# TheShinning/gps-sdr-sim

Hardware: AMD Instinct MI355X
Metric: IQ MSamples/s (and × real-time) at 2.6 MS/s, 12 sats, -b 16; 1/2/4/8 GPU (higher is better)
Workload: dtype int64 phases + f16 x f16 -> f32 MFMA accumulate (exact integer sums)

## Files before the change

### gps-sdr-sim_amd/csrc/hip/gss_synth.hip

```cpp
#include <hip/hip_runtime.h>
#include <stdint.h>
#include <stdlib.h>
#include <string.h>
#include "gpssim_amd.h"
#include "../common/gss_phase.h"
#include "../common/gss_lin.h"

#define SYNTH_THREADS  256
#define SYNTH_WAVES    (SYNTH_THREADS / 64)
#define ANCHOR_THREADS 64
#define CHUNK_BYTES    128
#define CHUNK_PIECES   (CHUNK_BYTES / 16)
#define LUT_N          1024

struct lut_arg { int16_t sin512[512]; int16_t cos512[512]; };

__global__ __launch_bounds__(ANCHOR_THREADS) void gss_anchor_kernel(
    const gss_chan_blk_t *__restrict__ blk, const int32_t *__restrict__ nch,
    const double *__restrict__ carr_ck, int nblk, int nchp, int n_per_blk, int nseg, int nsegp,
    int seg_r, double *__restrict__ seg_carr, double *__restrict__ seg_code,
    uint32_t *__restrict__ seg_cnt, double *__restrict__ carr_end,
    const int32_t *__restrict__ blist)
{
    const int nsub = carr_ck ? GSS_NCK : 1;
// ... 322 lines not shown
            } else {
                bits = (bits << 2) | ((uint32_t)(i16 > 0) << 1) | (uint32_t)(q16 > 0);
                if ((sidx & 15) == 15) {
                    int nb = nsamp - (sidx & ~15);
                    uint32_t w32 = nb >= 16 ? bits : nb > 0 ? (bits >> 2 * (16 - nb)) << 2 * (16 - nb) : 0u;
                    mine[sidx >> 4] = __builtin_bswap32(w32);
                    bits = 0;
                }
            }
        }
        if (last_seg && full && (ch + 1) * SPC == len) {
#pragma unroll
            for (int k = 0; k < NCH; k++) {
                const uint32_t c = s_st[k][tid];
                bad |= (C[k] >= GSS_CA_SEQ_LEN_D && c == (19u | (29u << 5) | (59u << 10))) ? 1 : 0;
            }
        }
        const bool any_full = __any(full);
        if (any_full) {
            wave_sync_lds();
            for (int i = 0; i < CHUNK_PIECES; i++) {
                int src = (64 / CHUNK_PIECES) * i + lane / CHUNK_PIECES, piece = lane % CHUNK_PIECES;
                int src_full = __shfl(full ? 1 : 0, src);
                if (src_full) {
                    uint8_t *sdst = dst + (ptrdiff_t)(src - lane) * ((ptrdiff_t)seg_r * BPS4 / 4) +
                                    (size_t)ch * CHUNK_BYTES + piece * 16;
                    const uint32_t *sp = stg + src * (CHUNK_BYTES / 4) + piece * 4;
                    store16(sdst, make_uint4(sp[0], sp[1], sp[2], sp[3]));
                }
            }
            wave_sync_lds();
        }
        if (!full && nsamp > 0) {
            int nbytes = nsamp * BPS4 / 4;
            uint8_t *bp = dst + (size_t)ch * CHUNK_BYTES;
            const uint8_t *sp = (const uint8_t *)mine;
            for (int i = 0; i < nbytes; i++)
                bp[i] = sp[i];
        }
    }
    if (bad && status)
        atomicOr(status, bad);
}

#define LIN_THREADS 256
#define LIN_WAVES   (LIN_THREADS / 64)
#define LIN_STEPS   (GSS_LIN_SEG / 64)
#define LIN_CH      GSS_LIN_CH
#define CBW_PRE     2
#define CBW_CHIPS   3072
#define CAB_W       ((CBW_CHIPS + 96) / 32)
static_assert(LIN_STEPS % LIN_CH == 0 && (LIN_CH & (LIN_CH - 1)) == 0, "whole chunks");
#define LIN_SW_SGPRS 68
typedef _Float16 lin_half4 __attribute__((ext_vector_type(4)));
typedef _Float16 lin_half8 __attribute__((ext_vector_type(8)));
typedef float lin_f4 __attribute__((ext_vector_type(4)));
#define LIN_GS    2
#define LIN_MAGF  (12582912.0f + 64.0f * LIN_GS)
#define LIN_MAGB  0x4B400000u

struct alignas(16) lin_ct {
    uint64_t B;
    uint64_t D;
    int32_t g;
    int32_t gd;
    int32_t pos1;
    uint32_t flags;
    uint32_t q0, dq, tab;
    uint32_t wa;
    uint32_t na, nb;
    uint32_t wn;
    uint32_t g2;
    uint32_t A[5][2];
};
static_assert(offsetof(lin_ct, A) % 8 == 0, "lin_ct.A: 8-byte reads");

typedef gss_lin_row lin_seg;
typedef gss_lin_chan lin_chan;
static_assert(sizeof(lin_seg) == 32 && sizeof(lin_chan) == 32, "two 16-byte LDS reads each");

__global__ void gss_cab_kernel(const uint32_t *__restrict__ ca_bits, int n_ca,
                               uint32_t *__restrict__ cab)
{
    const int i = blockIdx.x * blockDim.x + threadIdx.x;
    if (i >= n_ca * CAB_W)
        return;
    const int row = i / CAB_W, j0 = (i - row * CAB_W) * 32 - 32;
    const uint32_t *cb = ca_bits + (size_t)row * GSS_CA_WORDS;
    uint32_t w = 0;
    for (int q = 0; q < 32; q++) {
        const int e = j0 + q, chip = ((e % GSS_CA_LEN) + GSS_CA_LEN) % GSS_CA_LEN;
        w |= (((cb[chip >> 5] >> (chip & 31)) & 1u) ^ 1u) << q;
    }
    cab[i] = w;
}

__global__ void gss_tw16_kernel(const uint32_t *__restrict__ cab, int n_ca, uint32_t w,
                                uint32_t *__restrict__ tw)
{
    const int i = blockIdx.x * blockDim.x + threadIdx.x;
    if (i >= n_ca * GSS_LIN_TWE * LIN_CH)
        return;
    const int row = i / (GSS_LIN_TWE * LIN_CH), r = i - row * (GSS_LIN_TWE * LIN_CH);
    const int E = r / LIN_CH, st = r % LIN_CH;
    const uint32_t j = min((uint32_t)(E + (int)(((uint32_t)st * w) >> 4) - GSS_LIN_CBW_PRE + 32),
                           (uint32_t)(32 * CAB_W - 64));
    const uint32_t *c = cab + (size_t)row * CAB_W;
    const uint32_t lin = __builtin_amdgcn_alignbit(c[(j >> 5) + 1], c[j >> 5], j & 31);
    tw[i] = __builtin_amdgcn_alignbit(lin, lin, (32u - j) & 31u);
}

struct lin_wsrc {
    const uint32_t *W;
};

__device__ __forceinline__ void lin_wissue(const lin_wsrc &w, uint32_t (&ws)[LIN_CH])
{
#pragma unroll
    for (int s = 0; s < LIN_CH; s++)
        ws[s] = w.W[s];
}

__device__ __forceinline__ void lin_wfence(const uint32_t (&ws)[LIN_CH])
{
    static_assert(LIN_CH == 16, "the fence below names 16 windows");
// ... 135 lines not shown
{
    const lin_ct &ta = T[k0], &tb = T[k0 + 1];
    uint64_t Pa = s_lane[k0 * 64 + lane] + ta.B, Pb = s_lane[(k0 + 1) * 64 + lane] + tb.B;
    const uint64_t Da = ta.D, Db = tb.D;
    const uint2 ga = *(const uint2 *)ta.A[cls], gb = *(const uint2 *)tb.A[cls];
    const lin_half8 A = __builtin_bit_cast(lin_half8, make_uint4(ga.x, ga.y, gb.x, gb.y));
    uint32_t na = ta.na, nb = ta.nb;
    asm volatile("" : "+v"(na), "+v"(nb));
    uint32_t wsa[LIN_CH], wsb[LIN_CH];
    lin_sw_take_a(wsa);
    lin_sw_take(wsb);
    if (k0 + 2 < nc || more)
        lin_sw_load2(tw, na, nb);
    uint32_t ea0 = 0, eb0 = 0;
#pragma unroll
    for (int s = 0; s < LIN_CH; s++) {
        uint32_t ta_, tb_;
        asm("v_lshrrev_b32_sdwa %0, %1, %2 dst_sel:DWORD dst_unused:UNUSED_PAD src0_sel:BYTE_3 "
            "src1_sel:DWORD" : "=v"(ta_) : "v"((uint32_t)Pa), "s"(wsa[s]));
        asm("v_lshrrev_b32_sdwa %0, %1, %2 dst_sel:DWORD dst_unused:UNUSED_PAD src0_sel:BYTE_3 "
            "src1_sel:DWORD" : "=v"(tb_) : "v"((uint32_t)Pb), "s"(wsb[s]));
        const uint32_t aa = __builtin_amdgcn_alignbit(ta_, (uint32_t)(Pa >> 32), 21) & M;
        const uint32_t ab = __builtin_amdgcn_alignbit(tb_, (uint32_t)(Pb >> 32), 21) & M;
        const uint32_t ea = *(const uint32_t *)((const char *)s_lut + aa);
        const uint32_t eb = *(const uint32_t *)((const char *)s_lut + ab);
        if (s & 1) {
            const uint4 bb = make_uint4(ea0, ea, eb0, eb);
            cq[s / 2] = __builtin_amdgcn_mfma_f32_16x16x32_f16(A, __builtin_bit_cast(lin_half8, bb),
                                                              FIRST ? c0 : cq[s / 2], 0, 0, 0);
        } else {
            ea0 = ea;
            eb0 = eb;
        }
        Pa += Da;
        Pb += Db;
    }
}

__device__ __forceinline__ lin_half4 lin_gain_operand(uint32_t gh, int lane)
{
    const uint32_t x = gh << ((lane & 1) * 16);
    const uint2 v = (lane & 2) ? make_uint2(0u, x) : make_uint2(x, 0u);
    return __builtin_bit_cast(lin_half4, v);
}

__host__ __device__ __forceinline__ uint32_t lin_f16_bits(int g)
{
    return (uint32_t)__builtin_bit_cast(uint16_t, (_Float16)(float)g);
}

__device__ __forceinline__ void lin_put(uint32_t *p, uint32_t v)
{
    __builtin_nontemporal_store(v, p);
}

extern "C" __device__ int gss_writelane(int, int, int) __asm("llvm.amdgcn.writelane.i32");

__device__ __forceinline__ uint32_t lin_ib(const lin_f4 (&cq)[LIN_CH / 2], int s)
{
    return __float_as_uint(cq[s / 2][2 * (s & 1)]);
}
__device__ __forceinline__ uint32_t lin_qb(const lin_f4 (&cq)[LIN_CH / 2], int s)
{
    return __float_as_uint(cq[s / 2][2 * (s & 1) + 1]);
}
__device__ __forceinline__ uint32_t lin_w16(const lin_f4 (&cq)[LIN_CH / 2], int s)
{
    const uint32_t pq = __builtin_amdgcn_perm(lin_qb(cq, s), lin_ib(cq, s), 0x06050201u);
    uint32_t r;
    asm("v_pk_add_u16 %0, %1, %2" : "=v"(r) : "v"(pq), "s"(0xC000C000u));
    return r;
}
__device__ __forceinline__ uint32_t lin_w8(const lin_f4 (&cq)[LIN_CH / 2], int s)
{
    constexpr uint32_t sh = 12u;
    uint32_t d = lin_ib(cq, s) >> sh;
    asm("v_lshrrev_b32_sdwa %0, %1, %2 dst_sel:BYTE_1 dst_unused:UNUSED_PRESERVE src0_sel:DWORD "
        "src1_sel:DWORD" : "+v"(d) : "v"(sh), "v"(lin_qb(cq, s)));
    return d;
}
__device__ __forceinline__ bool lin_ipos(const lin_f4 (&cq)[LIN_CH / 2], int s)
{
    return lin_ib(cq, s) >= LIN_MAGB + 128u * LIN_GS;
}
__device__ __forceinline__ bool lin_qpos(const lin_f4 (&cq)[LIN_CH / 2], int s)
{
    return lin_qb(cq, s) >= LIN_MAGB + 128u * LIN_GS;
}

template <int FMT, bool TAIL>
__device__ __forceinline__ void lin_store(const lin_f4 (&acc)[LIN_CH / 2], uint8_t *__restrict__ ob,
                                          int nb0, int lane, int n_per_blk)
{
    static_assert(FMT != 1 || LIN_CH == 16, "-b 1 packing assumes 16-step chunks");
    uint32_t pk[LIN_CH];
    pk[0] = 0;
#pragma unroll
    for (int s = 0; s < LIN_CH; s++) {
        const int nb = nb0 + s * 64, p = nb + lane;
        const bool in = !TAIL || p < n_per_blk;
        if (FMT == 16) {
            pk[s] = lin_w16(acc, s);
        } else if (FMT == 8) {
            const uint32_t v = lin_w8(acc, s);
            if (!TAIL)
                asm volatile("global_store_short %0, %1, %2 offset:%3"
// ... 35 lines not shown
        }
    }
    if (FMT == 16) {
        __builtin_amdgcn_sched_barrier(0);
        if (!TAIL) {
            uint32_t *base = (uint32_t *)ob + nb0;
            const uint32_t off = (uint32_t)lane * 4u;
#pragma unroll
            for (int s = 0; s < LIN_CH; s++)
                asm volatile("global_store_dword %0, %1, %2 offset:%3 nt"
                             : : "v"(off), "v"(pk[s]), "s"(base + (s >> 4) * 1024),
                               "i"((s & 15) * 256) : "memory");
        } else {
#pragma unroll
            for (int s = 0; s < LIN_CH; s++) {
                const int p = nb0 + s * 64 + lane;
                if (!TAIL || p < n_per_blk)
                    lin_put(((uint32_t *)ob) + p, pk[s]);
            }
        }
    }
}

__device__ __forceinline__ void lin_patch_fix(lin_f4 (&cq)[LIN_CH / 2],
                                              const gss_lin_t *__restrict__ Lk, int nb0, int lane)
{
    for (int j = 0; j < GSS_NPATCH; j++) {
        const int pp = Lk->ppos[j];
        if (pp >= nb0 + 64 * LIN_CH)
            break;
        if (pp < nb0)
            continue;
        const int q = pp - nb0;
        const int64_t d = lane == (q & 63) ? Lk->pdelta[j] : 0;
        const int di = (int)((uint32_t)d << 10) >> 10;
        const float fi = (float)(di * LIN_GS), fq = (float)((int)((d - di) >> 22) * LIN_GS);
        const int sq = __builtin_amdgcn_readfirstlane(q >> 6);
#pragma unroll
        for (int s = 0; s < LIN_CH; s++) {
            const float m = s == sq ? 1.0f : 0.0f;
            cq[s / 2][2 * (s & 1)] = __builtin_fmaf(m, fi, cq[s / 2][2 * (s & 1)]);
            cq[s / 2][2 * (s & 1) + 1] = __builtin_fmaf(m, fq, cq[s / 2][2 * (s & 1) + 1]);
        }
    }
}


#define LIN_MINB 4
template <int FMT>
__global__ __launch_bounds__(LIN_THREADS, LIN_MINB) __attribute__((amdgpu_num_sgpr(LIN_SW_SGPRS)))
void gss_lin_kernel(
    const gss_lin_t *__restrict__ lin, const gss_chan_blk_t *__restrict__ blk,
    const int32_t *__restrict__ nch, const int32_t *__restrict__ fast,
    const uint32_t *__restrict__ cab, const uint32_t *__restrict__ tw,
    const uint4 *__restrict__ lut16, int n_per_blk, int wg_per_blk,
    uint8_t *__restrict__ out, size_t block_bytes)
{
    __shared__ alignas(16) int32_t s_lut[1024];
    __shared__ uint64_t s_lane[GSS_MAXCH * 64];
    __shared__ lin_ct s_ct[LIN_WAVES][GSS_MAXCH];
    __shared__ alignas(16) lin_seg s_seg[LIN_WAVES][GSS_MAXCH];
    __shared__ alignas(16) lin_chan s_chan[GSS_MAXCH];
    const int b = blockIdx.x / wg_per_blk;
    const int w = blockIdx.x - b * wg_per_blk;
    if (!fast[b])
        return;
    const int tid = threadIdx.x, lane = tid & 63;
    const int wave = __builtin_amdgcn_readfirstlane(tid >> 6);
    static_assert(sizeof(s_lut) == LIN_THREADS * sizeof(uint4), "one 16-byte copy per thread");
    const uint4 lutv = lut16[tid];
    const gss_lin_t *L = lin + (size_t)b * GSS_MAXCH;
    const int nc = nch[b];
#pragma unroll
    for (int j = 0; j < GSS_MAXCH / LIN_WAVES; j++) {
        const int k = wave + j * LIN_WAVES;
        if (k < nc)
            s_lane[k * 64 + lane] = gss_lin_lane(L[k].xs, L[k].zs, (uint32_t)lane);
    }
    {
        const int rk = lane & (GSS_MAXCH - 1), rj = lane / GSS_MAXCH;
        static_assert(LIN_WAVES * GSS_MAXCH == 64 && LIN_WAVES == 4, "one row per lane, 4 parts");
        const int rn0 = (w * LIN_WAVES + rj) * (64 * LIN_STEPS);
        if (rk < nc && rn0 < n_per_blk) {
            const gss_lin_t *Lk = L + rk;
            lin_seg &r = s_seg[rj][rk];
            if (wave == 0) {
                r.x = gss_lin_row_x(Lk->x0, Lk->xs, (uint64_t)rn0);
                r.z = gss_lin_row_z(Lk->z0, Lk->zs, (uint64_t)rn0);
            } else if (wave == 1) {
                gss_lin_row g;
                gss_lin_row_gain(&g, Lk->gpos, Lk->gval, GSS_NGC, rn0);
                r.g01 = g.g01;
                r.pos1 = g.pos1;
            } else if (wave == 2) {
                r.npatch = gss_lin_row_npatch(Lk->ppos, GSS_NPATCH, rn0);
                r.pad = 0;
            } else if (rj == 0) {
                s_chan[rk] = gss_lin_chan_of(Lk->xs, Lk->zs,
                                             (uint32_t)blk[(size_t)b * GSS_MAXCH + rk].ca_tbl);
            }
        }
    }
    ((uint4 *)s_lut)[tid] = lutv;
    (void)cab;
    __syncthreads();
    uint32_t M = 0xFFCu;
    asm volatile("" : "+v"(M));
    const uint32_t cls = lin_pair_cls(lane);
    lin_f4 c0 = lin_f4{LIN_MAGF, LIN_MAGF, LIN_MAGF, LIN_MAGF};
    asm volatile("" : "+v"(c0));
    const int sg = w * LIN_WAVES + wave;
    const int n0 = sg * (64 * LIN_STEPS);
    if (n0 >= n_per_blk)
        return;
    lin_ct *T = s_ct[wave];
    uint8_t *ob = out + (size_t)b * block_bytes;
    bool sw_ahead = false;
    uint64_t xb = 0, zb = 0, xs10 = 0, zs10 = 0;
    int32_t pos1 = INT32_MAX;
    uint32_t pflag = 0, gh0 = 0, gh1 = 0;
    uint32_t trow = 0, wa_next = 0;
    int g_after = -1;
    if (lane < nc) {
        const lin_chan ck = s_chan[lane];
        const lin_seg sk = s_seg[wave][lane];
        xb = sk.x;
        zb = sk.z;
        xs10 = ck.xs << 10;
        zs10 = ck.zs << 10;
        static_assert(64 * LIN_CH == 1024, "one chunk = 2^10 samples");
        pos1 = sk.pos1;
        pflag = sk.npatch != 0 ? 2u : 0u;
        const int g0 = (int)(int16_t)(sk.g01 & 0xFFFF), g1 = sk.g01 >> 16;
        gh0 = lin_f16_bits(g0 * LIN_GS);
        gh1 = lin_f16_bits(g1 * LIN_GS);
        lin_ct &t = T[lane];
        t.D = ck.d;
        t.gd = g1 - g0;
        t.pos1 = sk.pos1;
        t.dq = ck.dq;
        t.tab = ck.tab;
        t.A[4][0] = 0;
        t.A[4][1] = 0;
        trow = ck.tab * GSS_LIN_TWE;
        wa_next = (trow + min((uint32_t)(zb >> 50), (uint32_t)(GSS_LIN_TWE - 1))) *
                  (uint32_t)(LIN_CH * sizeof(uint32_t));
    }

    const int nc_blk = nc;
    for (int c = 0; c < LIN_STEPS / LIN_CH; c++) {
        int nc = nc_blk;
        asm volatile("" : "+s"(nc));
        const int nb0 = n0 + c * (64 * LIN_CH);
        if (nb0 >= n_per_blk)
            break;
        const bool after = pos1 <= nb0;
        const bool chg = pos1 < nb0 + 64 * LIN_CH;
        const uint32_t my_flags = (chg && !after ? 1u : 0u) | pflag;
        const uint64_t zn = zb + zs10;
        const uint32_t my_wa = wa_next;
        const uint32_t my_wn = (trow + min((uint32_t)(zn >> 50), (uint32_t)(GSS_LIN_TWE - 1))) *
                               (uint32_t)(LIN_CH * sizeof(uint32_t));
        if (lane < nc) {
            lin_ct &t = T[lane];
            t.B = (xb & ~0xFFFFFFFFull) | (uint32_t)(zb >> GSS_LIN_CSH);
            t.flags = my_flags;
            t.wa = my_wa;
            t.wn = my_wn;
            if ((int)after != g_after) {
                g_after = (int)after;
                const uint32_t gh = after ? gh1 : gh0;
                t.A[0][0] = gh;         t.A[0][1] = 0;
                t.A[1][0] = gh << 16;   t.A[1][1] = 0;
                t.A[2][0] = 0;          t.A[2][1] = gh;
                t.A[3][0] = 0;          t.A[3][1] = gh << 16;
                t.g2 = gh | (gh << 16);
            }
        }
        wa_next = my_wn;
        xb += xs10;
        zb = zn;
        const uint32_t wa0 = (uint32_t)__builtin_amdgcn_readlane((int)my_wa, 0);
        const uint32_t wa1r = (uint32_t)__builtin_amdgcn_readlane((int)my_wa, 1);
        const uint32_t wn0 = (uint32_t)__builtin_amdgcn_readlane((int)my_wn, 0);
        const uint32_t wn1r = (uint32_t)__builtin_amdgcn_readlane((int)my_wn, 1);
        const uint32_t wa1 = nc > 1 ? wa1r : wa0, wn1 = nc > 1 ? wn1r : wn0;
        {
            const uint32_t wa2 = (uint32_t)__builtin_amdgcn_update_dpp(0, (int)my_wa, 0x102, 0xF,
                                                                       0xF, true);
            const uint32_t wa3 = (uint32_t)__builtin_amdgcn_update_dpp(0, (int)my_wa, 0x103, 0xF,
                                                                       0xF, true);
            if (lane < nc) {
                const bool in2 = lane + 2 < nc, in3 = lane + 3 < nc;
                T[lane].na = in2 ? wa2 : wn0;
                T[lane].nb = in3 ? wa3 : in2 ? wa2 : wn1;
            }
        }
        const uint64_t fmask = __builtin_amdgcn_ballot_w64(my_flags != 0);
        wave_sync_lds();
        lin_f4 acc[LIN_CH / 2];
        if (nc > 0 && !sw_ahead)
            lin_sw_load2(tw, wa0, wa1);
        const bool more = c + 1 < LIN_STEPS / LIN_CH && nb0 + 64 * LIN_CH < n_per_blk;
        int k0 = 0;
        if (nc >= 2) {
            lin_sw_pair<true>(acc, c0, T, 0, nc, lane, s_lane, M, s_lut, tw, cls, more);
            k0 = 2;
        } else {
#pragma unroll
            for (int s = 0; s < LIN_CH / 2; s++) {
                lin_f4 v = c0;
                asm volatile("" : "+v"(v));
                acc[s] = v;
            }
        }
#pragma unroll
        for (int p = 1; p < GSS_MAXCH / 2; p++) {
            if (2 * p + 1 >= nc)
                break;
            lin_sw_pair<false>(acc, c0, T, 2 * p, nc, lane, s_lane, M, s_lut, tw, cls, more);
            k0 = 2 * p + 2;
        }
        if (k0 < nc) {
            uint32_t ws[LIN_CH], wb[LIN_CH];
            lin_sw_take_a(ws);
            lin_sw_take(wb);
            (void)wb;
            if (more)
                lin_sw_load2(tw, wn0, wn1);
            lin_sw_steps(acc, T[k0], k0, lane, s_lane, M, s_lut, ws);
            k0 = nc;
        }
        sw_ahead = nc > 0 && more;
        for (int k = k0; k < nc; k++) {
            const lin_ct &t = T[k];
            const uint64_t B = t.B, D = t.D;
            const uint2 a2 = *(const uint2 *)t.A[lane & 3];
            lin_channel_chunk_m<false>(acc, c0, s_lane[k * 64 + lane] + B, D, lin_wsrc_of(t, tw), M,
                                       __builtin_bit_cast(lin_half4, a2), 0, 0, s_lut);
        }
        for (uint64_t fm = fmask; fm; fm &= fm - 1) {
            const int k = __builtin_amdgcn_readfirstlane((int)__builtin_ctzll(fm));
            const lin_ct &t = T[k];
            const uint64_t B = t.B, D = t.D;
            const uint32_t fl = __builtin_amdgcn_readfirstlane(t.flags);
            if (__builtin_expect(fl & 1u, 0)) {
                uint32_t l2 = (uint32_t)lane;
                asm volatile("" : "+v"(l2));
                lin_channel_chunk_m<true>(acc, c0, s_lane[k * 64 + l2] + B, D, lin_wsrc_of(t, tw), M,
                                          lin_gain_operand(lin_f16_bits(t.gd * LIN_GS), (int)l2), t.pos1,
                                          nb0 + (int)l2, s_lut);
            }
            if (__builtin_expect(fl & 2u, 0))
                lin_patch_fix(acc, L + k, nb0, lane);
        }
        wave_sync_lds();
        if (nb0 + 64 * LIN_CH <= n_per_blk)
            lin_store<FMT, false>(acc, ob, nb0, lane, n_per_blk);
        else
            lin_store<FMT, true>(acc, ob, nb0, lane, n_per_blk);
    }
}


struct gss_dev {
    int ordinal;
    int seg_r = 1024;
    struct anchor_set {
        double *carr = nullptr, *code = nullptr;
        uint32_t *cnt = nullptr;
        size_t cap = 0;
    } set[2];
    static constexpr int RING = 256;
    hipEvent_t ev_a[RING][2], ev_b[RING][2];
    hipEvent_t ev_l[RING][2];
    int n_a = 0, n_b = 0, n_l = 0;
    lut_arg lut;
    uint4 *d_lut16 = nullptr;
    void *h_in = nullptr; size_t h_in_cap = 0;
    void *d_out = nullptr; size_t d_out_cap = 0;
    double *d_cend = nullptr; size_t d_cend_cap = 0;
    uint32_t *d_cbw = nullptr; size_t d_cbw_cap = 0;
    int32_t *d_status = nullptr;
    hipStream_t aux = nullptr;
    hipEvent_t ev_in = nullptr, ev_fb = nullptr;
};

extern "C" int gss_fail(int code, const char *fmt, ...);

#define HIP_TRY(x)                                                                           \
    do {                                                                                     \
        hipError_t e_ = (x);                                                                 \
        if (e_ != hipSuccess)                                                                \
            return gss_fail(GSS_E_HIP, "HIP error %s at %s:%d", hipGetErrorString(e_),      \
                            __FILE__, __LINE__);                                             \
    } while (0)

#define GSS_STR2(x) #x
#define GSS_STR(x) GSS_STR2(x)
extern "C" int gss_dev_ordinal(const gss_dev *d) { return d->ordinal; }

extern "C" const char *gss_build_info(void)
{
    return "lin_mfma=2 lin_ch=" GSS_STR(LIN_CH) " lin_swin=3 spec_k=" GSS_STR(GSS_SPEC_K)
           " arch=gfx950";
}


extern "C" void gss_run_pool_prewarm(int dev);

extern "C" int gss_dev_open(gss_dev **out, int ordinal)
{
    *out = nullptr;
    int count = 0;
    if (hipGetDeviceCount(&count) != hipSuccess || count <= 0)
        return gss_fail(GSS_E_NODEV, "no HIP device visible");
    if (ordinal < 0 || ordinal >= count)
        return gss_fail(GSS_E_ARG, "device ordinal %d out of range (%d devices)", ordinal, count);
    HIP_TRY(hipSetDevice(ordinal));
    gss_dev *d = new gss_dev();
    d->ordinal = ordinal;
    const char *r = getenv("GSS_SEG_R");
    if (r && atoi(r) >= 256 && atoi(r) % 256 == 0)
        d->seg_r = atoi(r);
    for (int i = 0; i < gss_dev::RING; i++)
        for (int j = 0; j < 2; j++) {
            HIP_TRY(hipEventCreate(&d->ev_a[i][j]));
            HIP_TRY(hipEventCreate(&d->ev_b[i][j]));
            HIP_TRY(hipEventCreate(&d->ev_l[i][j]));
        }
    int32_t s[512], c[512];
    gss_lut(s, c);
    for (int i = 0; i < 512; i++) {
        d->lut.sin512[i] = (int16_t)s[i];
        d->lut.cos512[i] = (int16_t)c[i];
    }
    {
        uint32_t packed[1024];
        for (int i = 0; i < 512; i++) {
            const uint32_t v = lin_f16_bits(c[i]) | (lin_f16_bits(s[i]) << 16);
            packed[i] = v;
            packed[512 + i] = v ^ 0x80008000u;
        }
        HIP_TRY(hipMalloc(&d->d_lut16, sizeof(packed)));
        HIP_TRY(hipMemcpy(d->d_lut16, packed, sizeof(packed), hipMemcpyHostToDevice));
    }
    HIP_TRY(hipMalloc(&d->d_status, sizeof(int32_t)));
    int prio_lo = 0, prio_hi = 0;
    HIP_TRY(hipDeviceGetStreamPriorityRange(&prio_lo, &prio_hi));
    HIP_TRY(hipStreamCreateWithPriority(&d->aux, hipStreamNonBlocking, prio_hi));
    HIP_TRY(hipEventCreateWithFlags(&d->ev_in, hipEventDisableTiming));
    HIP_TRY(hipEventCreateWithFlags(&d->ev_fb, hipEventDisableTiming));
    gss_run_pool_prewarm(ordinal);
    *out = d;
    return 0;
}

extern "C" void gss_run_pool_drain(int dev);

extern "C" int gss_dev_close(gss_dev *d)
{
    if (!d) return 0;
    (void)hipSetDevice(d->ordinal);
    gss_run_pool_drain(d->ordinal);
    for (auto &a : d->set) {
        (void)hipFree(a.carr);
        (void)hipFree(a.code);
        (void)hipFree(a.cnt);
    }
    if (d->aux) (void)hipStreamDestroy(d->aux);
    if (d->ev_in) (void)hipEventDestroy(d->ev_in);
    if (d->ev_fb) (void)hipEventDestroy(d->ev_fb);
    void *bufs[] = {d->h_in, d->d_out, d->d_cend, d->d_cbw, d->d_lut16, d->d_status};
    for (void *p : bufs)
        (void)hipFree(p);
    for (int i = 0; i < gss_dev::RING; i++)
        for (int j = 0; j < 2; j++) {
// ... 97 lines not shown
                                 const int32_t *nch, int nch_max, const double *carr_ck,
                                 int nblk, int n_per_blk, double *carr_end, void *stream)
{
    return anchor_launch(d, set, blk, nch, nch_max, carr_ck, nblk, n_per_blk, carr_end, nullptr,
                         d->seg_r, stream);
}

static int render_launch(gss_dev *d, int set, const gss_chan_blk_t *blk, const int32_t *nch,
                         int nch_max, const uint32_t *ca_bits, const uint32_t *nav, int nblk,
                         int n_per_blk, int fmt, void *out, int32_t *status,
                         const int32_t *blist, int R, void *stream)
{
    if (!d || !blk || !nch || !ca_bits || !out || nblk <= 0 || n_per_blk <= 0 || set < 0 ||
        set > 1)
        return gss_fail(GSS_E_ARG, "invalid render arguments");
    const size_t bb = gss_block_bytes(n_per_blk, fmt);
    if (bb == 0)
        return gss_fail(GSS_E_ARG, "invalid format %d for %d samples/block", fmt, n_per_blk);
    const int nseg = nseg_of(n_per_blk, R), nsegp = nsegp_of(n_per_blk, R);
    const gss_dev::anchor_set &a = d->set[set];
    if ((size_t)nblk * GSS_MAXCH * (size_t)nsegp > a.cap)
        return gss_fail(GSS_E_STATE, "anchor set %d holds no Stage A output of this size", set);
    const int nchp = nch_max < 1 ? 1 : nch_max;
    if (nchp > GSS_MAXCH)
        return gss_fail(GSS_E_ARG, "nch_max %d > %d", nch_max, GSS_MAXCH);
    synth_fn fn = pick_kernel(fmt, nchp);
    if (!fn)
        return gss_fail(GSS_E_ARG, "no kernel for fmt=%d nch=%d", fmt, nchp);
    HIP_TRY(hipSetDevice(d->ordinal));
    hipStream_t st = (hipStream_t)stream;
    hipEvent_t *ev = d->ev_b[d->n_b % gss_dev::RING];
    d->n_b++;
    const int wg_per_blk = (nseg + SYNTH_THREADS - 1) / SYNTH_THREADS;
    HIP_TRY(hipEventRecord(ev[0], st));
    hipLaunchKernelGGL(fn, dim3(nblk * wg_per_blk), dim3(SYNTH_THREADS), 0, st, blk, nch, ca_bits,
                       nav, a.carr, a.code, a.cnt, d->lut, n_per_blk, nseg, nsegp, R, wg_per_blk,
                       (uint8_t *)out, bb, status, blist);
    HIP_TRY(hipGetLastError());
    HIP_TRY(hipEventRecord(ev[1], st));
    return 0;
}

extern "C" int gss_render_device(gss_dev *d, int set, const gss_chan_blk_t *blk,
                                 const int32_t *nch, int nch_max, const uint32_t *ca_bits,
                                 int n_ca, const uint32_t *nav, int n_nav, int nblk,
                                 int n_per_blk, int fmt, void *out, int32_t *status, void *stream)
{
    (void)n_ca; (void)n_nav;
    return render_launch(d, set, blk, nch, nch_max, ca_bits, nav, nblk, n_per_blk, fmt, out,
                         status, nullptr, d->seg_r, stream);
}

typedef void (*lin_fn)(const gss_lin_t *, const gss_chan_blk_t *, const int32_t *,
                       const int32_t *, const uint32_t *, const uint32_t *, const uint4 *, int,
                       int, uint8_t *, size_t);

static lin_fn pick_lin(int fmt)
{
    switch (fmt) {
    case 16: return gss_lin_kernel<16>;
    case 8: return gss_lin_kernel<8>;
    case 1: return gss_lin_kernel<1>;
    default: return nullptr;
    }
}

extern "C" int gss_synth_lin_device(gss_dev *d, const gss_chan_blk_t *blk, const int32_t *nch,
                                    int nch_max, const gss_lin_t *lin, const int32_t *fast,
                                    const int32_t *fb_list, int n_fb, const double *carr_ck,
                                    const uint32_t *ca_bits, int n_ca, const uint32_t *nav,
                                    int n_nav, int nblk, int n_per_blk, int fmt, void *out,
                                    int32_t *status, void *stream)
{
    (void)n_nav;
    if (!d || !blk || !nch || !lin || !fast || !ca_bits || !out || nblk <= 0 || n_per_blk <= 0 ||
        n_ca <= 0 || n_fb < 0 || n_fb > nblk || (n_fb > 0 && !fb_list))
        return gss_fail(GSS_E_ARG, "invalid synth_lin arguments");
    const size_t bb = gss_block_bytes(n_per_blk, fmt);
    if (bb == 0)
        return gss_fail(GSS_E_ARG, "invalid format %d for %d samples/block", fmt, n_per_blk);
    const int nchp = nch_max < 1 ? 1 : nch_max;
    if (nchp > GSS_MAXCH)
        return gss_fail(GSS_E_ARG, "nch_max %d > %d", nch_max, GSS_MAXCH);
    lin_fn fn = pick_lin(fmt);
    if (!fn)
        return gss_fail(GSS_E_ARG, "no fast kernel for fmt=%d nch=%d", fmt, nchp);
    HIP_TRY(hipSetDevice(d->ordinal));
    hipStream_t st = (hipStream_t)stream;
    const size_t ncbw = (size_t)n_ca * CAB_W, ntw = (size_t)n_ca * GSS_LIN_TWE * LIN_CH;
    const size_t tw_off = (ncbw + 63) & ~(size_t)63;
    if ((tw_off + ntw) * sizeof(uint32_t) > d->d_cbw_cap) {
        (void)hipFree(d->d_cbw);
        d->d_cbw = nullptr;
        d->d_cbw_cap = 0;
        HIP_TRY(hipMalloc(&d->d_cbw, (tw_off + ntw) * sizeof(uint32_t)));
        d->d_cbw_cap = (tw_off + ntw) * sizeof(uint32_t);
    }
    hipLaunchKernelGGL(gss_cab_kernel, dim3((unsigned)((ncbw + 255) / 256)), dim3(256), 0, st,
                       ca_bits, n_ca, d->d_cbw);
    HIP_TRY(hipGetLastError());
    hipLaunchKernelGGL(gss_tw16_kernel, dim3((unsigned)((ntw + 255) / 256)), dim3(256), 0, st,
                       (const uint32_t *)d->d_cbw, n_ca, gss_lin_wstep16(n_per_blk),
                       d->d_cbw + tw_off);
    HIP_TRY(hipGetLastError());
    const int segs = (n_per_blk + 64 * LIN_STEPS - 1) / (64 * LIN_STEPS);
    const int wg_per_blk = (segs + LIN_WAVES - 1) / LIN_WAVES;
    if (n_fb > 0) {
        HIP_TRY(hipEventRecord(d->ev_in, st));
        HIP_TRY(hipStreamWaitEvent(d->aux, d->ev_in, 0));
        const int R = 256;
        int rc = anchor_launch(d, 0, blk, nch, nch_max, carr_ck, n_fb, n_per_blk, nullptr,
                               fb_list, R, d->aux);
        if (rc) return rc;
        rc = render_launch(d, 0, blk, nch, nch_max, ca_bits, nav, n_fb, n_per_blk, fmt, out,
                           status, fb_list, R, d->aux);
        if (rc) return rc;
        HIP_TRY(hipEventRecord(d->ev_fb, d->aux));
    }
    hipEvent_t *ev = d->ev_l[d->n_l % gss_dev::RING];
    d->n_l++;
    HIP_TRY(hipEventRecord(ev[0], st));
    hipLaunchKernelGGL(fn, dim3((unsigned)nblk * wg_per_blk), dim3(LIN_THREADS), 0, st, lin,
                       blk, nch, fast, d->d_cbw, d->d_cbw + tw_off, (const uint4 *)d->d_lut16,
                       n_per_blk, wg_per_blk, (uint8_t *)out, bb);
    HIP_TRY(hipGetLastError());
    HIP_TRY(hipEventRecord(ev[1], st));
    if (n_fb > 0)
        HIP_TRY(hipStreamWaitEvent(st, d->ev_fb, 0));
    return 0;
}

extern "C" int gss_synth_device(gss_dev *d, const gss_chan_blk_t *blk, const int32_t *nch,
                                int nch_max, const double *carr_ck, const uint32_t *ca_bits,
                                int n_ca,
                                const uint32_t *nav, int n_nav, int nblk, int n_per_blk, int fmt,
                                void *out, double *carr_end, int32_t *status, void *stream)
{
    if (!d || !blk || !nch || !ca_bits || !out || nblk <= 0 || n_per_blk <= 0)
        return gss_fail(GSS_E_ARG, "invalid synth arguments");
    if (gss_block_bytes(n_per_blk, fmt) == 0)
        return gss_fail(GSS_E_ARG, "invalid format %d for %d samples/block", fmt, n_per_blk);
    int rc = gss_anchor_device(d, 0, blk, nch, nch_max, carr_ck, nblk, n_per_blk, carr_end,
                               stream);
    if (rc) return rc;
    return gss_render_device(d, 0, blk, nch, nch_max, ca_bits, n_ca, nav, n_nav, nblk, n_per_blk,
                             fmt, out, status, stream);
}

static int ring_avg(hipEvent_t (*ev)[2], int n, double *avg)
{
    const int cnt = n < gss_dev::RING ? n : gss_dev::RING;
    double acc = 0.0;
    if (cnt > 0) {
        HIP_TRY(hipEventSynchronize(ev[(n - 1) % gss_dev::RING][1]));
        for (int i = 0; i < cnt; i++) {
            hipEvent_t *e = ev[(n - 1 - i) % gss_dev::RING];
            float t = 0.f;
            HIP_TRY(hipEventElapsedTime(&t, e[0], e[1]));
            acc += t;
        }
        acc /= cnt;
    }
    *avg = acc;
    return 0;
}

extern "C" int gss_dev_timing(gss_dev *d, int reset, int *n, float *ckpt_ms, float *synth_ms)
{
    if (!d) return gss_fail(GSS_E_ARG, "null device");
    if (reset) {
        d->n_a = d->n_b = d->n_l = 0;
        return 0;
    }
    double a = 0.0, b = 0.0;
    int rc = ring_avg(d->ev_a, d->n_a, &a);
    if (rc) return rc;
    rc = ring_avg(d->ev_b, d->n_b, &b);
// ... 175 lines not shown
```

Measured before the change: 514,400.

## Let each workgroup process multiple segment passes per wave via GSS_LIN_SPW

Adds an outer loop so each wave can process up to four consecutive segment passes, with per-pass row state (x/z phases, gain, patch counts) precomputed into an enlarged LDS table. The workgroup count per block shrinks by the chosen factor, so the per-workgroup setup (LUT copy, lane table, channel info) is spread over more work. The factor is read from an environment variable and defaults to one, so by default the launch geometry is unchanged. It also drops unused lin_ct fields and the unused cab argument. The enlarged LDS footprint and the extra loop add some register and LDS pressure.

```diff
diff --git a/gps-sdr-sim_amd/csrc/hip/gss_synth.hip b/gps-sdr-sim_amd/csrc/hip/gss_synth.hip
--- a/gps-sdr-sim_amd/csrc/hip/gss_synth.hip
+++ b/gps-sdr-sim_amd/csrc/hip/gss_synth.hip
@@ -398,6 +398,7 @@
 #define CAB_W       ((CBW_CHIPS + 96) / 32)
 static_assert(LIN_STEPS % LIN_CH == 0 && (LIN_CH & (LIN_CH - 1)) == 0, "whole chunks");
 #define LIN_SW_SGPRS 68
+#define LIN_SPW_MAX 4
 typedef _Float16 lin_half4 __attribute__((ext_vector_type(4)));
 typedef _Float16 lin_half8 __attribute__((ext_vector_type(8)));
 typedef float lin_f4 __attribute__((ext_vector_type(4)));
@@ -408,15 +409,11 @@
 struct alignas(16) lin_ct {
     uint64_t B;
     uint64_t D;
-    int32_t g;
     int32_t gd;
     int32_t pos1;
     uint32_t flags;
-    uint32_t q0, dq, tab;
     uint32_t wa;
     uint32_t na, nb;
-    uint32_t wn;
-    uint32_t g2;
     uint32_t A[5][2];
 };
 static_assert(offsetof(lin_ct, A) % 8 == 0, "lin_ct.A: 8-byte reads");
@@ -658,6 +655,12 @@
 __device__ __forceinline__ void lin_put(uint32_t *p, uint32_t v)
 {
     __builtin_nontemporal_store(v, p);
+}
+
+__device__ __forceinline__ uint64_t lin_uniform64(uint64_t v)
+{
+    return (uint64_t)(uint32_t)__builtin_amdgcn_readfirstlane((int)v) |
+           (uint64_t)(uint32_t)__builtin_amdgcn_readfirstlane((int)(v >> 32)) << 32;
 }
 
 extern "C" __device__ int gss_writelane(int, int, int) __asm("llvm.amdgcn.writelane.i32");
@@ -799,15 +802,16 @@
 void gss_lin_kernel(
     const gss_lin_t *__restrict__ lin, const gss_chan_blk_t *__restrict__ blk,
     const int32_t *__restrict__ nch, const int32_t *__restrict__ fast,
-    const uint32_t *__restrict__ cab, const uint32_t *__restrict__ tw,
-    const uint4 *__restrict__ lut16, int n_per_blk, int wg_per_blk,
+    const uint32_t *__restrict__ tw,
+    const uint4 *__restrict__ lut16, int n_per_blk, int wg_per_blk, int spw,
     uint8_t *__restrict__ out, size_t block_bytes)
 {
     __shared__ alignas(16) int32_t s_lut[1024];
     __shared__ uint64_t s_lane[GSS_MAXCH * 64];
     __shared__ lin_ct s_ct[LIN_WAVES][GSS_MAXCH];
-    __shared__ alignas(16) lin_seg s_seg[LIN_WAVES][GSS_MAXCH];
+    __shared__ alignas(16) lin_seg s_seg[LIN_SPW_MAX][LIN_WAVES][GSS_MAXCH];
     __shared__ alignas(16) lin_chan s_chan[GSS_MAXCH];
+    constexpr int pass_n = LIN_WAVES * 64 * LIN_STEPS;
     const int b = blockIdx.x / wg_per_blk;
     const int w = blockIdx.x - b * wg_per_blk;
     if (!fast[b])
@@ -827,21 +831,49 @@
     {
         const int rk = lane & (GSS_MAXCH - 1), rj = lane / GSS_MAXCH;
         static_assert(LIN_WAVES * GSS_MAXCH == 64 && LIN_WAVES == 4, "one row per lane, 4 parts");
-        const int rn0 = (w * LIN_WAVES + rj) * (64 * LIN_STEPS);
+        const int rn0 = (w * spw * LIN_WAVES + rj) * (64 * LIN_STEPS);
         if (rk < nc && rn0 < n_per_blk) {
             const gss_lin_t *Lk = L + rk;
-            lin_seg &r = s_seg[rj][rk];
             if (wave == 0) {
-                r.x = gss_lin_row_x(Lk->x0, Lk->xs, (uint64_t)rn0);
-                r.z = gss_lin_row_z(Lk->z0, Lk->zs, (uint64_t)rn0);
+                const uint64_t x0 = Lk->x0, xs = Lk->xs, z0 = Lk->z0, zs = Lk->zs;
+#pragma unroll
+                for (int i = 0, n = rn0; i < LIN_SPW_MAX; i++, n += pass_n) {
+                    if (i >= spw || n >= n_per_blk)
+                        break;
+                    lin_seg &r = s_seg[i][rj][rk];
+                    r.x = gss_lin_row_x(x0, xs, (uint64_t)n);
+                    r.z = gss_lin_row_z(z0, zs, (uint64_t)n);
+                }
             } else if (wave == 1) {
-                gss_lin_row g;
-                gss_lin_row_gain(&g, Lk->gpos, Lk->gval, GSS_NGC, rn0);
-                r.g01 = g.g01;
-                r.pos1 = g.pos1;
+                int32_t gp[GSS_NGC], gv[GSS_NGC];
+#pragma unroll
+                for (int q = 0; q < GSS_NGC; q++) {
+                    gp[q] = Lk->gpos[q];
+                    gv[q] = Lk->gval[q];
+                }
+#pragma unroll
+                for (int i = 0, n = rn0; i < LIN_SPW_MAX; i++, n += pass_n) {
+                    if (i >= spw || n >= n_per_blk)
+                        break;
+                    lin_seg &r = s_seg[i][rj][rk];
+                    gss_lin_row g;
+                    gss_lin_row_gain(&g, gp, gv, GSS_NGC, n);
+                    r.g01 = g.g01;
+                    r.pos1 = g.pos1;
+                }
             } else if (wave == 2) {
-                r.npatch = gss_lin_row_npatch(Lk->ppos, GSS_NPATCH, rn0);
-                r.pad = 0;
+                int32_t pp[GSS_NPATCH];
+#pragma unroll
+                for (int q = 0; q < GSS_NPATCH; q++)
+                    pp[q] = Lk->ppos[q];
+#pragma unroll
+                for (int i = 0, n = rn0; i < LIN_SPW_MAX; i++, n += pass_n) {
+                    if (i >= spw || n >= n_per_blk)
+                        break;
+                    lin_seg &r = s_seg[i][rj][rk];
+                    r.npatch = gss_lin_row_npatch(pp, GSS_NPATCH, n);
+                    r.pad = 0;
+                }
             } else if (rj == 0) {
                 s_chan[rk] = gss_lin_chan_of(Lk->xs, Lk->zs,
                                              (uint32_t)blk[(size_t)b * GSS_MAXCH + rk].ca_tbl);
@@ -849,163 +881,169 @@
         }
     }
     ((uint4 *)s_lut)[tid] = lutv;
-    (void)cab;
     __syncthreads();
     uint32_t M = 0xFFCu;
     asm volatile("" : "+v"(M));
     const uint32_t cls = lin_pair_cls(lane);
     lin_f4 c0 = lin_f4{LIN_MAGF, LIN_MAGF, LIN_MAGF, LIN_MAGF};
     asm volatile("" : "+v"(c0));
-    const int sg = w * LIN_WAVES + wave;
-    const int n0 = sg * (64 * LIN_STEPS);
-    if (n0 >= n_per_blk)
-        return;
     lin_ct *T = s_ct[wave];
     uint8_t *ob = out + (size_t)b * block_bytes;
-    bool sw_ahead = false;
-    uint64_t xb = 0, zb = 0, xs10 = 0, zs10 = 0;
-    int32_t pos1 = INT32_MAX;
-    uint32_t pflag = 0, gh0 = 0, gh1 = 0;
-    uint32_t trow = 0, wa_next = 0;
-    int g_after = -1;
+    uint64_t xs10 = 0, zs10 = 0;
+    uint32_t trow = 0;
     if (lane < nc) {
         const lin_chan ck = s_chan[lane];
-        const lin_seg sk = s_seg[wave][lane];
-        xb = sk.x;
-        zb = sk.z;
         xs10 = ck.xs << 10;
         zs10 = ck.zs << 10;
         static_assert(64 * LIN_CH == 1024, "one chunk = 2^10 samples");
-        pos1 = sk.pos1;
-        pflag = sk.npatch != 0 ? 2u : 0u;
-        const int g0 = (int)(int16_t)(sk.g01 & 0xFFFF), g1 = sk.g01 >> 16;
-        gh0 = lin_f16_bits(g0 * LIN_GS);
-        gh1 = lin_f16_bits(g1 * LIN_GS);
         lin_ct &t = T[lane];
         t.D = ck.d;
-        t.gd = g1 - g0;
-        t.pos1 = sk.pos1;
-        t.dq = ck.dq;
-        t.tab = ck.tab;
         t.A[4][0] = 0;
         t.A[4][1] = 0;
         trow = ck.tab * GSS_LIN_TWE;
-        wa_next = (trow + min((uint32_t)(zb >> 50), (uint32_t)(GSS_LIN_TWE - 1))) *
-                  (uint32_t)(LIN_CH * sizeof(uint32_t));
-    }
-
+    }
     const int nc_blk = nc;
-    for (int c = 0; c < LIN_STEPS / LIN_CH; c++) {
-        int nc = nc_blk;
-        asm volatile("" : "+s"(nc));
-        const int nb0 = n0 + c * (64 * LIN_CH);
-        if (nb0 >= n_per_blk)
-            break;
-        const bool after = pos1 <= nb0;
-        const bool chg = pos1 < nb0 + 64 * LIN_CH;
-        const uint32_t my_flags = (chg && !after ? 1u : 0u) | pflag;
-        const uint64_t zn = zb + zs10;
-        const uint32_t my_wa = wa_next;
-        const uint32_t my_wn = (trow + min((uint32_t)(zn >> 50), (uint32_t)(GSS_LIN_TWE - 1))) *
-                               (uint32_t)(LIN_CH * sizeof(uint32_t));
-        if (lane < nc) {
+    const int n_first = (w * spw * LIN_WAVES + wave) * (64 * LIN_STEPS);
+    int n_lim = min(n_per_blk, n_first + spw * pass_n);
+    uint64_t lines = (uint64_t)L;
+    asm volatile("" : "+v"(n_lim), "+v"(lines));
+    const lin_seg *seg = &s_seg[0][wave][lane];
+    for (int n0 = n_first; n0 < __builtin_amdgcn_readfirstlane(n_lim);
+         n0 += pass_n, seg += LIN_WAVES * GSS_MAXCH) {
+        bool sw_ahead = false;
+        uint64_t xb = 0, zb = 0;
+        int32_t pos1 = INT32_MAX;
+        uint32_t pflag = 0, gh0 = 0, gh1 = 0;
+        uint32_t wa_next = 0;
+        int g_after = -1;
+        if (lane < nc_blk) {
+            const lin_seg sk = *seg;
+            xb = sk.x;
+            zb = sk.z;
+            pos1 = sk.pos1;
+            pflag = sk.npatch != 0 ? 2u : 0u;
+            const int g0 = (int)(int16_t)(sk.g01 & 0xFFFF), g1 = sk.g01 >> 16;
+            gh0 = lin_f16_bits(g0 * LIN_GS);
+            gh1 = lin_f16_bits(g1 * LIN_GS);
             lin_ct &t = T[lane];
-            t.B = (xb & ~0xFFFFFFFFull) | (uint32_t)(zb >> GSS_LIN_CSH);
-            t.flags = my_flags;
-            t.wa = my_wa;
-            t.wn = my_wn;
-            if ((int)after != g_after) {
-                g_after = (int)after;
-                const uint32_t gh = after ? gh1 : gh0;
-                t.A[0][0] = gh;         t.A[0][1] = 0;
-                t.A[1][0] = gh << 16;   t.A[1][1] = 0;
-                t.A[2][0] = 0;          t.A[2][1] = gh;
-                t.A[3][0] = 0;          t.A[3][1] = gh << 16;
-                t.g2 = gh | (gh << 16);
-            }
-        }
-        wa_next = my_wn;
-        xb += xs10;
-        zb = zn;
-        const uint32_t wa0 = (uint32_t)__builtin_amdgcn_readlane((int)my_wa, 0);
-        const uint32_t wa1r = (uint32_t)__builtin_amdgcn_readlane((int)my_wa, 1);
-        const uint32_t wn0 = (uint32_t)__builtin_amdgcn_readlane((int)my_wn, 0);
-        const uint32_t wn1r = (uint32_t)__builtin_amdgcn_readlane((int)my_wn, 1);
-        const uint32_t wa1 = nc > 1 ? wa1r : wa0, wn1 = nc > 1 ? wn1r : wn0;
-        {
-            const uint32_t wa2 = (uint32_t)__builtin_amdgcn_update_dpp(0, (int)my_wa, 0x102, 0xF,
-                                                                       0xF, true);
-            const uint32_t wa3 = (uint32_t)__builtin_amdgcn_update_dpp(0, (int)my_wa, 0x103, 0xF,
-                                                                       0xF, true);
+            t.gd = g1 - g0;
+            t.pos1 = sk.pos1;
+            wa_next = (trow + min((uint32_t)(zb >> 50), (uint32_t)(GSS_LIN_TWE - 1))) *
+                      (uint32_t)(LIN_CH * sizeof(uint32_t));
+        }
+        for (int c = 0; c < LIN_STEPS / LIN_CH; c++) {
+            int nc = nc_blk;
+            asm volatile("" : "+s"(nc));
+            const int nb0 = n0 + c * (64 * LIN_CH);
+            if (nb0 >= n_per_blk)
+                break;
+            const bool after = pos1 <= nb0;
+            const bool chg = pos1 < nb0 + 64 * LIN_CH;
+            const uint32_t my_flags = (chg && !after ? 1u : 0u) | pflag;
+            const uint64_t zn = zb + zs10;
+            const uint32_t my_wa = wa_next;
+            const uint32_t my_wn = (trow + min((uint32_t)(zn >> 50), (uint32_t)(GSS_LIN_TWE - 1))) *
+                                   (uint32_t)(LIN_CH * sizeof(uint32_t));
             if (lane < nc) {
-                const bool in2 = lane + 2 < nc, in3 = lane + 3 < nc;
-                T[lane].na = in2 ? wa2 : wn0;
-                T[lane].nb = in3 ? wa3 : in2 ? wa2 : wn1;
-            }
-        }
-        const uint64_t fmask = __builtin_amdgcn_ballot_w64(my_flags != 0);
-        wave_sync_lds();
-        lin_f4 acc[LIN_CH / 2];
-        if (nc > 0 && !sw_ahead)
-            lin_sw_load2(tw, wa0, wa1);
-        const bool more = c + 1 < LIN_STEPS / LIN_CH && nb0 + 64 * LIN_CH < n_per_blk;
-        int k0 = 0;
-        if (nc >= 2) {
-            lin_sw_pair<true>(acc, c0, T, 0, nc, lane, s_lane, M, s_lut, tw, cls, more);
-            k0 = 2;
-        } else {
-#pragma unroll
-            for (int s = 0; s < LIN_CH / 2; s++) {
-                lin_f4 v = c0;
-                asm volatile("" : "+v"(v));
-                acc[s] = v;
-            }
-        }
-#pragma unroll
-        for (int p = 1; p < GSS_MAXCH / 2; p++) {
-            if (2 * p + 1 >= nc)
-                break;
-            lin_sw_pair<false>(acc, c0, T, 2 * p, nc, lane, s_lane, M, s_lut, tw, cls, more);
-            k0 = 2 * p + 2;
-        }
-        if (k0 < nc) {
-            uint32_t ws[LIN_CH], wb[LIN_CH];
-            lin_sw_take_a(ws);
-            lin_sw_take(wb);
-            (void)wb;
-            if (more)
-                lin_sw_load2(tw, wn0, wn1);
-            lin_sw_steps(acc, T[k0], k0, lane, s_lane, M, s_lut, ws);
-            k0 = nc;
-        }
-        sw_ahead = nc > 0 && more;
-        for (int k = k0; k < nc; k++) {
-            const lin_ct &t = T[k];
-            const uint64_t B = t.B, D = t.D;
-            const uint2 a2 = *(const uint2 *)t.A[lane & 3];
-            lin_channel_chunk_m<false>(acc, c0, s_lane[k * 64 + lane] + B, D, lin_wsrc_of(t, tw), M,
-                                       __builtin_bit_cast(lin_half4, a2), 0, 0, s_lut);
-        }
-        for (uint64_t fm = fmask; fm; fm &= fm - 1) {
-            const int k = __builtin_amdgcn_readfirstlane((int)__builtin_ctzll(fm));
-            const lin_ct &t = T[k];
-            const uint64_t B = t.B, D = t.D;
-            const uint32_t fl = __builtin_amdgcn_readfirstlane(t.flags);
-            if (__builtin_expect(fl & 1u, 0)) {
-                uint32_t l2 = (uint32_t)lane;
-                asm volatile("" : "+v"(l2));
-                lin_channel_chunk_m<true>(acc, c0, s_lane[k * 64 + l2] + B, D, lin_wsrc_of(t, tw), M,
-                                          lin_gain_operand(lin_f16_bits(t.gd * LIN_GS), (int)l2), t.pos1,
-                                          nb0 + (int)l2, s_lut);
-            }
-            if (__builtin_expect(fl & 2u, 0))
-                lin_patch_fix(acc, L + k, nb0, lane);
-        }
-        wave_sync_lds();
-        if (nb0 + 64 * LIN_CH <= n_per_blk)
-            lin_store<FMT, false>(acc, ob, nb0, lane, n_per_blk);
-        else
-            lin_store<FMT, true>(acc, ob, nb0, lane, n_per_blk);
+                lin_ct &t = T[lane];
+                t.B = (xb & ~0xFFFFFFFFull) | (uint32_t)(zb >> GSS_LIN_CSH);
+                t.flags = my_flags;
+                t.wa = my_wa;
+                if ((int)after != g_after) {
+                    g_after = (int)after;
+                    const uint32_t gh = after ? gh1 : gh0;
+                    t.A[0][0] = gh;         t.A[0][1] = 0;
+                    t.A[1][0] = gh << 16;   t.A[1][1] = 0;
+                    t.A[2][0] = 0;          t.A[2][1] = gh;
+                    t.A[3][0] = 0;          t.A[3][1] = gh << 16;
+                }
+            }
+            wa_next = my_wn;
+            xb += xs10;
+            zb = zn;
+            const uint32_t wa0 = (uint32_t)__builtin_amdgcn_readlane((int)my_wa, 0);
+            const uint32_t wa1r = (uint32_t)__builtin_amdgcn_readlane((int)my_wa, 1);
+            const uint32_t wn0 = (uint32_t)__builtin_amdgcn_readlane((int)my_wn, 0);
+            const uint32_t wn1r = (uint32_t)__builtin_amdgcn_readlane((int)my_wn, 1);
+            const uint32_t wa1 = nc > 1 ? wa1r : wa0, wn1 = nc > 1 ? wn1r : wn0;
+            {
+                const uint32_t wa2 = (uint32_t)__builtin_amdgcn_update_dpp(0, (int)my_wa, 0x102,
+                                                                           0xF, 0xF, true);
+                const uint32_t wa3 = (uint32_t)__builtin_amdgcn_update_dpp(0, (int)my_wa, 0x103,
+                                                                           0xF, 0xF, true);
+                if (lane < nc) {
+                    const bool in2 = lane + 2 < nc, in3 = lane + 3 < nc;
+                    T[lane].na = in2 ? wa2 : wn0;
+                    T[lane].nb = in3 ? wa3 : in2 ? wa2 : wn1;
+                }
+            }
+            const uint64_t fmask = __builtin_amdgcn_ballot_w64(my_flags != 0);
+            wave_sync_lds();
+            lin_f4 acc[LIN_CH / 2];
+            if (nc > 0 && !sw_ahead)
+                lin_sw_load2(tw, wa0, wa1);
+            const bool more = c + 1 < LIN_STEPS / LIN_CH && nb0 + 64 * LIN_CH < n_per_blk;
+            int k0 = 0;
+            if (nc >= 2) {
+                lin_sw_pair<true>(acc, c0, T, 0, nc, lane, s_lane, M, s_lut, tw, cls, more);
+                k0 = 2;
+            } else {
+#pragma unroll
+                for (int s = 0; s < LIN_CH / 2; s++) {
+                    lin_f4 v = c0;
+                    asm volatile("" : "+v"(v));
+                    acc[s] = v;
+                }
+            }
+#pragma unroll
+            for (int p = 1; p < GSS_MAXCH / 2; p++) {
+                if (2 * p + 1 >= nc)
+                    break;
+                lin_sw_pair<false>(acc, c0, T, 2 * p, nc, lane, s_lane, M, s_lut, tw, cls, more);
+                k0 = 2 * p + 2;
+            }
+            if (k0 < nc) {
+                uint32_t ws[LIN_CH], wb[LIN_CH];
+                lin_sw_take_a(ws);
+                lin_sw_take(wb);
+                (void)wb;
+                if (more)
+                    lin_sw_load2(tw, wn0, wn1);
+                lin_sw_steps(acc, T[k0], k0, lane, s_lane, M, s_lut, ws);
+                k0 = nc;
+            }
+            sw_ahead = nc > 0 && more;
+            for (int k = k0; k < nc; k++) {
+                const lin_ct &t = T[k];
+                const uint64_t B = t.B, D = t.D;
+                const uint2 a2 = *(const uint2 *)t.A[lane & 3];
+                lin_channel_chunk_m<false>(acc, c0, s_lane[k * 64 + lane] + B, D,
+                                           lin_wsrc_of(t, tw), M,
+                                           __builtin_bit_cast(lin_half4, a2), 0, 0, s_lut);
+            }
+            for (uint64_t fm = fmask; fm; fm &= fm - 1) {
+                const int k = __builtin_amdgcn_readfirstlane((int)__builtin_ctzll(fm));
+                const lin_ct &t = T[k];
+                const uint64_t B = t.B, D = t.D;
+                const uint32_t fl = __builtin_amdgcn_readfirstlane(t.flags);
+                if (__builtin_expect(fl & 1u, 0)) {
+                    uint32_t l2 = (uint32_t)lane;
+                    asm volatile("" : "+v"(l2));
+                    lin_channel_chunk_m<true>(acc, c0, s_lane[k * 64 + l2] + B, D,
+                                              lin_wsrc_of(t, tw), M,
+                                              lin_gain_operand(lin_f16_bits(t.gd * LIN_GS),
+                                                               (int)l2),
+                                              t.pos1, nb0 + (int)l2, s_lut);
+                }
+                if (__builtin_expect(fl & 2u, 0))
+                    lin_patch_fix(acc, (const gss_lin_t *)lin_uniform64(lines) + k, nb0, lane);
+            }
+            wave_sync_lds();
+            if (nb0 + 64 * LIN_CH <= n_per_blk)
+                lin_store<FMT, false>(acc, ob, nb0, lane, n_per_blk);
+            else
+                lin_store<FMT, true>(acc, ob, nb0, lane, n_per_blk);
+        }
     }
 }
 
@@ -1013,6 +1051,7 @@
 struct gss_dev {
     int ordinal;
     int seg_r = 1024;
+    int lin_spw = 1;
     struct anchor_set {
         double *carr = nullptr, *code = nullptr;
         uint32_t *cnt = nullptr;
@@ -1070,6 +1109,9 @@
     const char *r = getenv("GSS_SEG_R");
     if (r && atoi(r) >= 256 && atoi(r) % 256 == 0)
         d->seg_r = atoi(r);
+    const char *spw = getenv("GSS_LIN_SPW");
+    if (spw && atoi(spw) >= 1 && atoi(spw) <= LIN_SPW_MAX)
+        d->lin_spw = atoi(spw);
     for (int i = 0; i < gss_dev::RING; i++)
         for (int j = 0; j < 2; j++) {
             HIP_TRY(hipEventCreate(&d->ev_a[i][j]));
@@ -1273,8 +1315,8 @@
 }
 
 typedef void (*lin_fn)(const gss_lin_t *, const gss_chan_blk_t *, const int32_t *,
-                       const int32_t *, const uint32_t *, const uint32_t *, const uint4 *, int,
-                       int, uint8_t *, size_t);
+                       const int32_t *, const uint32_t *, const uint4 *, int, int, int, uint8_t *,
+                       size_t);
 
 static lin_fn pick_lin(int fmt)
 {
@@ -1325,7 +1367,8 @@
                        d->d_cbw + tw_off);
     HIP_TRY(hipGetLastError());
     const int segs = (n_per_blk + 64 * LIN_STEPS - 1) / (64 * LIN_STEPS);
-    const int wg_per_blk = (segs + LIN_WAVES - 1) / LIN_WAVES;
+    const int spw = d->lin_spw;
+    const int wg_per_blk = (segs + LIN_WAVES * spw - 1) / (LIN_WAVES * spw);
     if (n_fb > 0) {
         HIP_TRY(hipEventRecord(d->ev_in, st));
         HIP_TRY(hipStreamWaitEvent(d->aux, d->ev_in, 0));
@@ -1342,8 +1385,8 @@
     d->n_l++;
     HIP_TRY(hipEventRecord(ev[0], st));
     hipLaunchKernelGGL(fn, dim3((unsigned)nblk * wg_per_blk), dim3(LIN_THREADS), 0, st, lin,
-                       blk, nch, fast, d->d_cbw, d->d_cbw + tw_off, (const uint4 *)d->d_lut16,
-                       n_per_blk, wg_per_blk, (uint8_t *)out, bb);
+                       blk, nch, fast, d->d_cbw + tw_off, (const uint4 *)d->d_lut16, n_per_blk,
+                       wg_per_blk, spw, (uint8_t *)out, bb);
     HIP_TRY(hipGetLastError());
     HIP_TRY(hipEventRecord(ev[1], st));
     if (n_fb > 0)
```

Result: no change. 516,600 (median of 3 runs) (+0.4%).
